# argmaxinc/DiffusionKit

Hardware: AMD Instinct MI355X
Metric: images/sec (whole node) FLUX.1-schnell 1024x1024 4-step (higher is better)
Workload: dtype bf16; 1 GPU; flux-schnell-1024: latent 128x128, 4 Euler steps, cfg_weight 0.0, text tokens 256, batch 1 image per GPU per step, + VAE decode to uint8; parallelism=dp1 (independent images, weight broadcast at load)

## Files before the change

### diffusionkit_amd/csrc/attention.hip

```cpp
#include "dk_kernels.h"

extern int g_dk_attn_mode;

static thread_local void* g_attn_ws = nullptr;
static thread_local size_t g_attn_ws_bytes = 0;
void dk_set_attention_workspace(void* ws, size_t bytes) { g_attn_ws = ws, g_attn_ws_bytes = ws ? bytes : 0; }
void* dk_get_attention_workspace() { return g_attn_ws; }
size_t dk_get_attention_workspace_bytes() { return g_attn_ws_bytes; }

int dk_launch_attention(const AttnParams& p_in, hipStream_t stream) {
  AttnParams p = p_in;
  if (p.bal_ws == nullptr) p.bal_ws = g_attn_ws;
  DK_REQUIRE(p.D == 128 || p.D == 64, "head_dim must be 64 or 128");
  DK_REQUIRE(p.S > 0 && p.B > 0 && p.H > 0, "empty attention");
  DK_REQUIRE(p.ld % 8 == 0 && p.ldo % 4 == 0, "row strides must keep 16-byte alignment");
  const long blocks5 = (long)p.B * p.H * ((p.S + 255) / 256);
  const bool long5 = p.D == 128 && (p.S >= 2048 || (p.S >= 1024 && blocks5 * 4 >= 3L * dk_device_cu_count()));
  int mode = p.bias != nullptr ? 4 : g_dk_attn_mode < 0 ? (long5 ? 10 : 4) : g_dk_attn_mode;
  if (mode == 10 && !dk_attention5_eligible(p)) mode = 9;
  dk_prof_begin(2, 4.0 * (double)p.B * p.H * (double)p.S * (double)p.S * p.D, stream);
  int rc = 0;
  switch (mode) {
    case 4: rc = dk_launch_attention2(p, 4, stream); break;
    case 9:
      rc = p.D == 128 ? dk_launch_attention4(p, stream) : dk_launch_attention2(p, 4, stream);
      break;
    case 10: rc = dk_launch_attention5(p, stream); break;
    default: DK_REQUIRE(false, "unknown attention variant (4: lean kernel, 9: phase-alternating kernel, 10: one-wave-per-SIMD kernel)");
  }
  dk_prof_end(stream);
  if (rc) return rc;
  DK_CHECK_HIP(hipGetLastError());
  if (p.O8 != nullptr && !((mode == 9 || mode == 10) && p.D == 128)) {
    Mx8Out o8{p.O8, p.O8_scales, p.o8_ld, p.o8_nblk, 0, p.B * p.S, 0, 0};
    return dk_launch_quantize_mx8(p.O, p.ldo, p.B * p.S, 0, p.B * p.S, p.H * p.D, o8, stream);
  }
  return 0;
}
```

### diffusionkit_amd/csrc/attention5.hip

```cpp
#include "dk_kernels.h"

typedef __attribute__((address_space(3))) char a5_lds_char;
typedef unsigned int u32x16 __attribute__((ext_vector_type(16)));
typedef unsigned int u32x8 __attribute__((ext_vector_type(8)));

#define A5_LDS_BYTES 131072

template <bool QFUSE>
__global__ __launch_bounds__(256, 1) void dk_attn5_fwd_kernel(AttnParams p) {
  constexpr int D = 128;
  extern __shared__ __attribute__((aligned(16))) char smem[];
  if ((unsigned)(size_t)(a5_lds_char*)smem != 0u) __builtin_trap();
  const int tid = threadIdx.x, lane = tid & 63;
  const int wave = __builtin_amdgcn_readfirstlane(tid >> 6);
  const int hi = lane >> 5, l31 = lane & 31;
  const int S = p.S;
  const int nq = (S + 255) / 256;
  auto xcd_contiguous = [](int bid, int nwg) {
    const int xcd = bid & 7, q = nwg >> 3, r = nwg & 7;
    return (xcd < r ? xcd * (q + 1) : r * (q + 1) + (xcd - r) * q) + (bid >> 3);
  };
  int t, part = 0, job = -1;
  if ((int)blockIdx.x < p.a5_whole) {
    t = xcd_contiguous(blockIdx.x, p.a5_whole);
  } else {
    job = xcd_contiguous(blockIdx.x - p.a5_whole, gridDim.x - p.a5_whole);
    t = p.a5_whole + job / p.a5_split;
    part = job % p.a5_split;
  }
  const unsigned row_bytes = (unsigned)p.ld * 2u;
  const int qblock = t % nq, head = (t / nq) % p.H, b = t / (nq * p.H);
  const int q0 = qblock * 256 + wave * 64;
  const int ng = S / 256, nparts = job < 0 ? 1 : p.a5_split;
  const int g_lo = (part * ng) / nparts, g_hi = ((part + 1) * ng) / nparts;
  const int tile0 = 4 * g_lo, nt = 4 * (g_hi - g_lo);

  const bf16_t* Qb = p.Q + (size_t)b * S * p.ld + head * D;
  const char* Kb = (const char*)(p.K + ((size_t)b * S + (size_t)tile0 * 64) * p.ld + head * D);
  const char* Vb = (const char*)(p.V + ((size_t)b * S + (size_t)tile0 * 64) * p.ld + head * D);

  u32x8 kaddr;
  const unsigned kr_base = (unsigned)(l31 * 256 + ((hi ^ (l31 & 15)) << 4));
#pragma unroll
  for (int kk = 0; kk < 8; ++kk) kaddr[kk] = kr_base ^ (unsigned)(kk << 5);
  const int x16 = (lane >> 4) & 1, p16 = lane & 15;
  u32x2 vaddr;
#pragma unroll
  for (int par = 0; par < 2; ++par) vaddr[par] = (unsigned)(65536 + x16 * 2048 + ((4 * (hi ^ x16) + (p16 >> 2)) ^ (2 * par + x16)) * 32 + (p16 & 3) * 8);
  u32x4 dk, dv;
#pragma unroll
  for (int i = 0; i < 4; ++i) {
    const int pi = 4 * wave + i;
    const int row = 4 * pi + (lane >> 4);
    dk[i] = (unsigned)row * row_bytes + (unsigned)(((lane & 15) ^ (row & 15)) << 4);
    const int dg = pi >> 1, hf = pi & 1;
    const int kl = (hf * 32 + (lane >> 1)) ^ (((dg & 1) << 2) | (dg & 3));
    dv[i] = (unsigned)kl * row_bytes + (unsigned)((2 * dg + (lane & 1)) << 4);
  }
  const u32x4 rK = {(unsigned)(size_t)Kb, (unsigned)((size_t)Kb >> 32) & 0xffffu, 0xffffffffu, 0x00020000u};
  const u32x4 rV = {(unsigned)(size_t)Vb, (unsigned)((size_t)Vb >> 32) & 0xffffu, 0xffffffffu, 0x00020000u};
  asm volatile(
#include "attention5_dma.inc"
      :
      : [tileb] "s"(64 * (int)row_bytes), [dbase] "s"(wave * 4096), "{v[248:251]}"(dk), "{v[252:255]}"(dv), "{s[40:43]}"(rK), "{s[44:47]}"(rV)
      : "s48", "s49", "s50", "s55", "m0", "scc", "memory");

  u32x16 qv[4];
#pragma unroll
  for (int qb = 0; qb < 2; ++qb) {
    bf16x8 qf[D / 16];
    const int qrow = min(q0 + qb * 32 + l31, S - 1);
    const bf16_t* qp = Qb + (size_t)qrow * p.ld + hi * 8;
#pragma unroll
    for (int kk = 0; kk < D / 16; ++kk) qf[kk] = *(const bf16x8*)(qp + kk * 16);
    if (QFUSE) {
      bf16x8 wv[D / 16];
      f32x4 t0[D / 16], t1[D / 16];
      if (p.qn_a != nullptr) {
        const bf16_t* w = (qrow < p.qn_split ? p.qn_a : p.qn_b) + hi * 8;
#pragma unroll
        for (int kk = 0; kk < D / 16; ++kk) wv[kk] = *(const bf16x8*)(w + kk * 16);
      }
      if (p.q_rope != nullptr) {
        const float* tab = p.q_rope + ((size_t)qrow * (D / 2) + hi * 4) * 2;
#pragma unroll
        for (int kk = 0; kk < D / 16; ++kk) t0[kk] = *(const f32x4*)(tab + kk * 16), t1[kk] = *(const f32x4*)(tab + kk * 16 + 4);
      }
      float v[D / 16][8];
#pragma unroll
      for (int kk = 0; kk < D / 16; ++kk)
#pragma unroll
        for (int e = 0; e < 8; ++e) v[kk][e] = (float)qf[kk][e];
      if (p.qn_a != nullptr) {
        float ss = 0.f;
#pragma unroll
        for (int kk = 0; kk < D / 16; ++kk)
#pragma unroll
          for (int e = 0; e < 8; ++e) ss += v[kk][e] * v[kk][e];
        ss += __shfl_xor(ss, 32, 64);
        const float r = rsqrtf(ss / (float)D + p.qn_eps);
#pragma unroll
        for (int kk = 0; kk < D / 16; ++kk)
#pragma unroll
          for (int e = 0; e < 8; ++e) v[kk][e] = round_bf16(v[kk][e] * r * (float)wv[kk][e]);
      }
      if (p.q_rope != nullptr) {
#pragma unroll
        for (int kk = 0; kk < D / 16; ++kk) {
          const float cs[8] = {t0[kk][0], t0[kk][1], t0[kk][2], t0[kk][3], t1[kk][0], t1[kk][1], t1[kk][2], t1[kk][3]};
#pragma unroll
          for (int i = 0; i < 4; ++i) {
            const float c = cs[2 * i], sn = cs[2 * i + 1], xe = v[kk][2 * i], xo = v[kk][2 * i + 1];
            v[kk][2 * i] = c * xe - sn * xo;
            v[kk][2 * i + 1] = sn * xe + c * xo;
          }
        }
      }
#pragma unroll
      for (int kk = 0; kk < D / 16; ++kk)
#pragma unroll
        for (int e = 0; e < 8; ++e) qf[kk][e] = (__bf16)v[kk][e];
    }
#pragma unroll
    for (int kk = 0; kk < D / 16; ++kk) {
      const u32x4 w4 = __builtin_bit_cast(u32x4, qf[kk]);
#pragma unroll
      for (int r = 0; r < 4; ++r) qv[(qb * 8 + kk) >> 2][((qb * 8 + kk) & 3) * 4 + r] = w4[r];
    }
  }

  const int scale_bits = __float_as_int(p.scale);

  f32x16 o[2][4];
  u32x2 lsum, mcv;
  asm volatile(
#include "attention5_asm.inc"
      : "={v[0:15]}"(o[0][0]), "={v[16:31]}"(o[0][1]), "={v[32:47]}"(o[0][2]), "={v[48:63]}"(o[0][3]), "={v[64:79]}"(o[1][0]), "={v[80:95]}"(o[1][1]),
        "={v[96:111]}"(o[1][2]), "={v[112:127]}"(o[1][3]), "={v[226:227]}"(lsum), "={v[224:225]}"(mcv), "+{v[128:143]}"(qv[0]), "+{v[144:159]}"(qv[1]), "+{v[160:175]}"(qv[2]),
        "+{v[176:191]}"(qv[3])
      : [koff] "s"(64 * (int)row_bytes), [voff] "s"(0), [tileb] "s"(64 * (int)row_bytes), [scale] "s"(scale_bits), [ntrip] "s"((nt - 8) / 4), [dbase] "s"(wave * 4096), "{v[238:245]}"(kaddr),
        "{v[246:247]}"(vaddr), "{v[248:251]}"(dk), "{v[252:255]}"(dv), "{s[40:43]}"(rK), "{s[44:47]}"(rV)
      :
#include "attention5_clobbers.inc"
  );

  int lane_t;
  asm volatile("v_mbcnt_lo_u32_b32 %0, -1, 0\n\tv_mbcnt_hi_u32_b32 %0, -1, %0" : "=v"(lane_t));
  {
    const int lane = lane_t, hi = lane >> 5, l31 = lane & 31;
#pragma unroll
  for (int qb = 0; qb < 2; ++qb) {
    const float l_run = __uint_as_float(lsum[qb]);
    const float inv = 1.0f / (l_run + __shfl_xor(l_run, 32, 64));
    const int q = q0 + qb * 32 + l31;
    if (p.O8 != nullptr) {
      const size_t orow = (size_t)b * S + min(q, S - 1);
#pragma unroll
      for (int dt = 0; dt < D / 32; ++dt) {
        float v[16], amax = 0.f;
#pragma unroll
        for (int e = 0; e < 16; ++e) {
          v[e] = round_bf16(o[qb][dt][e] * inv);
          amax = fmaxf(amax, fabsf(v[e]));
        }
        amax = fmaxf(amax, __shfl_xor(amax, 32, 64));
        const float ts = amax * (1.0f / 448.0f);
        unsigned e8 = (__float_as_uint(ts) + 0x7FFFFFu) >> 23;
        e8 = e8 < 1u ? 1u : (e8 > 254u ? 254u : e8);
        const float sc = __uint_as_float((254u - e8) << 23);
        if (q < S) {
          unsigned char* orow8 = p.O8 + orow * (size_t)p.o8_ld + head * D + dt * 32 + 4 * hi;
#pragma unroll
          for (int g4 = 0; g4 < 4; ++g4) {
            int w = 0;
            w = __builtin_amdgcn_cvt_pk_fp8_f32(v[4 * g4 + 0] * sc, v[4 * g4 + 1] * sc, w, false);
            w = __builtin_amdgcn_cvt_pk_fp8_f32(v[4 * g4 + 2] * sc, v[4 * g4 + 3] * sc, w, true);
            *(int*)(orow8 + 8 * g4) = w;
          }
          if (hi == 0) p.O8_scales[dk_mx_scale_index((unsigned)orow, (unsigned)(head * (D / 32) + dt), (unsigned)p.o8_nblk)] = (unsigned char)e8;
        }
      }
    }
  }
  if (p.O8 == nullptr) {
    a5_lds_char* const lds = (a5_lds_char*)0;
    const unsigned img = (unsigned)wave * 16384u;
#pragma unroll
    for (int qb = 0; qb < 2; ++qb) {
      const float l_run = __uint_as_float(lsum[qb]);
      const float inv = 1.0f / (l_run + __shfl_xor(l_run, 32, 64));
      const int r = qb * 32 + l31;
#pragma unroll
      for (int dt = 0; dt < D / 32; ++dt)
#pragma unroll
        for (int g4 = 0; g4 < 4; ++g4) {
          u32x2 w;
          w[0] = pack2bf(o[qb][dt][4 * g4 + 0] * inv, o[qb][dt][4 * g4 + 1] * inv);
          w[1] = pack2bf(o[qb][dt][4 * g4 + 2] * inv, o[qb][dt][4 * g4 + 3] * inv);
          *(__attribute__((address_space(3))) u32x2*)(lds + img + r * 256 + (((dt * 4 + g4) ^ (r & 15)) << 4) + hi * 8) = w;
        }
    }
    const int njobs = (int)gridDim.x - p.a5_whole;
    bf16_t* const ob = job < 0 ? p.O + ((size_t)b * S + q0) * p.ldo + head * D : (bf16_t*)p.a5_ws + ((size_t)job * 256 + wave * 64) * D;
    const size_t ldo = job < 0 ? (size_t)p.ldo : (size_t)D;
#pragma unroll
    for (int i = 0; i < 16; ++i) {
      const int r = 4 * i + (lane >> 4), pos = lane & 15;
      const u32x4 v = *(const __attribute__((address_space(3))) u32x4*)(lds + img + r * 256 + (pos << 4));
      if (q0 + r < S) *(u32x4*)(ob + (size_t)r * ldo + ((pos ^ (r & 15)) << 3)) = v;
    }
    if (job >= 0) {
      float* st = (float*)((char*)p.a5_ws + (size_t)njobs * 65536) + ((size_t)job * 256 + wave * 64) * 2;
#pragma unroll
      for (int qb = 0; qb < 2; ++qb) {
        const float l_run = __uint_as_float(lsum[qb]);
        const float l_row = l_run + __shfl_xor(l_run, 32, 64);
        if (hi == 0) *(f32x2*)(st + (qb * 32 + l31) * 2) = f32x2{__uint_as_float(mcv[qb]), l_row};
      }
    }
  }
  }
}

__global__ __launch_bounds__(256) void dk_attn5_merge_kernel(AttnParams p, int njobs) {
  constexpr int D = 128;
  const int blk = blockIdx.x >> 4, row = (blockIdx.x & 15) * 16 + (threadIdx.x >> 4), c8 = threadIdx.x & 15;
  const int nq = (p.S + 255) / 256;
  const int t = p.a5_whole + blk;
  const int qblock = t % nq, head = (t / nq) % p.H, b = t / (nq * p.H);
  const int q = qblock * 256 + row;
  const float* st = (const float*)((const char*)p.a5_ws + (size_t)njobs * 65536);
  float mc[4], l[4], mx = -3.0e38f;
  for (int i = 0; i < p.a5_split; ++i) {
    const f32x2 s2 = *(const f32x2*)(st + ((size_t)(blk * p.a5_split + i) * 256 + row) * 2);
    mc[i] = s2[0], l[i] = s2[1];
    mx = fmaxf(mx, mc[i]);
  }
  float acc[8] = {0.f, 0.f, 0.f, 0.f, 0.f, 0.f, 0.f, 0.f}, wsum = 0.f;
  for (int i = 0; i < p.a5_split; ++i) {
    const float w = l[i] * __builtin_amdgcn_exp2f(mc[i] - mx);
    const u32x4 v = *(const u32x4*)((const bf16_t*)p.a5_ws + ((size_t)(blk * p.a5_split + i) * 256 + row) * D + c8 * 8);
    wsum += w;
#pragma unroll
    for (int e = 0; e < 4; ++e) {
      float lo, hi2;
      unpack2bf(v[e], lo, hi2);
      acc[2 * e] += w * lo, acc[2 * e + 1] += w * hi2;
    }
  }
  const float inv = 1.0f / wsum;
  if (q < p.S) {
    u32x4 o;
#pragma unroll
    for (int e = 0; e < 4; ++e) o[e] = pack2bf(acc[2 * e] * inv, acc[2 * e + 1] * inv);
    *(u32x4*)(p.O + ((size_t)b * p.S + q) * p.ldo + head * D + c8 * 8) = o;
  }
}

int g_dk_attn5_split = -1;

bool dk_attention5_eligible(const AttnParams& p) {
  return p.D == 128 && p.bias == nullptr && p.S % 256 == 0 && p.S >= 12 * 64 && (size_t)p.S * p.ld * 2 < (1ull << 32);
}

int dk_launch_attention5(const AttnParams& p_in, hipStream_t stream) {
  DK_REQUIRE(dk_attention5_eligible(p_in), "attention5: head_dim 128, no score bias, S a multiple of 256 and >= 768");
  AttnParams p = p_in;
  const bool qfuse = p.qn_a != nullptr || p.q_rope != nullptr;
  if (qfuse) DK_REQUIRE(p.qn_a == nullptr || p.qn_b != nullptr, "qn_b missing (pass qn_a twice for one weight)");
  const int n_cu = dk_device_cu_count();
  const int nb = ((p.S + 255) / 256) * p.H * p.B;
  const int tail = nb % n_cu;
  int split = 1;
  if (tail > 0 && p.O8 == nullptr && g_dk_attn5_split != 0) {
    for (int s = 2; s <= 4 && split == 1; ++s) {
      if ((p.S / 256) / s < 3) break;
      if (g_dk_attn5_split > 0 ? s == g_dk_attn5_split : (tail * s <= n_cu && tail * s * 10 >= n_cu * 6)) split = s;
    }
    void* ws = dk_get_attention_workspace();
    if (split > 1 && (ws == nullptr || dk_get_attention_workspace_bytes() < (size_t)tail * split * (65536 + 2048))) split = 1;
    p.a5_ws = ws;
  }
  p.a5_split = split;
  p.a5_whole = split > 1 ? nb - tail : nb;
  const int njobs = split > 1 ? tail * split : 0;
  static DkDeviceOnce attr_once;
  if (attr_once.first()) {
    DK_CHECK_HIP(hipFuncSetAttribute((const void*)dk_attn5_fwd_kernel<true>, hipFuncAttributeMaxDynamicSharedMemorySize, A5_LDS_BYTES));
    DK_CHECK_HIP(hipFuncSetAttribute((const void*)dk_attn5_fwd_kernel<false>, hipFuncAttributeMaxDynamicSharedMemorySize, A5_LDS_BYTES));
    attr_once.mark();
  }
  if (qfuse)
    hipLaunchKernelGGL((dk_attn5_fwd_kernel<true>), dim3((unsigned)(p.a5_whole + njobs)), dim3(256), A5_LDS_BYTES, stream, p);
  else
    hipLaunchKernelGGL((dk_attn5_fwd_kernel<false>), dim3((unsigned)(p.a5_whole + njobs)), dim3(256), A5_LDS_BYTES, stream, p);
  if (njobs > 0) hipLaunchKernelGGL(dk_attn5_merge_kernel, dim3((unsigned)(tail * 16)), dim3(256), 0, stream, p, njobs);
  return 0;
}
```

### diffusionkit_amd/csrc/dk_kernels.h

```cpp
#pragma once
#include "../../include/dk_hip.h"
#include "dk_common.h"
#include "dk_ksplit.h"


struct GemmParams {
  const bf16_t* A;
  const bf16_t* W;
  bf16_t* C;
  const bf16_t* bias;
  const bf16_t* gate;
  const bf16_t* res;
  int M, N, K;
  int lda, ldc, ldr;
  int ldw;
  int a_seg_len, a_seg_stride;
  int c_seg_len, c_seg_stride;
  int r_seg_len, r_seg_stride;
  int gate_seg_len, gate_stride;
  float alpha;
  int epi;
  int conv;
  int cB, cH, cW, cC, ups;
  const bf16_t* zeros;
// ... 58 lines not shown
}

struct GemmF8Params {
  const unsigned char* A;
  const unsigned char* SA;
  const unsigned char* W;
  const float* wscale;
  void* C;
  const bf16_t* bias;
  const bf16_t* gate;
  const bf16_t* res;
  int M, N, K;
  int lda, ldw, ldc, ldr;
  int a_seg_len, a_seg_stride, a_row0;
  int sa_nblk;
  int c_seg_len, c_seg_stride;
  int r_seg_len, r_seg_stride;
  int gate_seg_len, gate_stride;
  int epi;
  int c_mx8;
  int n_split;
  void* C2;
  int ldc2, epi2, c2_mx8;
  unsigned char* SC;
  int sc_nblk, c_row0, sc_kb0;
  const bf16_t* kn_w;
  const float* kn_rope;
  int kn_col0, kn_col1, kn_D, kn_pos_off, kn_seg_len;
  float kn_eps;
  const bf16_t* qn_w;
  int qn_col0, qn_col1;
  void* workspace;
  size_t workspace_bytes;
};
bool dk_gemm256f8_eligible(const GemmF8Params& p);
int dk_launch_gemm256f8(const GemmF8Params& p, const GemmF8Params* p2, hipStream_t stream);
struct Mx8Out {
  unsigned char* out;
  unsigned char* scales;
  int ldo, n_blk128, row0, seg_len, seg_stride, col0;
};
int dk_launch_quantize_mx8(const bf16_t* x, int ldx, int x_seg_len, int x_seg_stride, int M, int h, const Mx8Out& o, hipStream_t stream);
int dk_launch_ln_modulate_mx8(const bf16_t* x, int ldx, int M, int h, const bf16_t* shift, const bf16_t* scale, int mod_stride, int seg_len,
                              int x_seg_len, int x_seg_stride, float eps, const Mx8Out& o, hipStream_t stream);
int dk_launch_ln_modulate2_mx8(const bf16_t* x0, int M0, const bf16_t* shift0, const bf16_t* scale0, int seg0, const Mx8Out& o0,
                               const bf16_t* x1, int M1, const bf16_t* shift1, const bf16_t* scale1, int seg1, const Mx8Out& o1, int ldx, int h,
                               int mod_stride, int x_seg_stride, float eps, hipStream_t stream);

void dk_prof_begin(int cls, double work, hipStream_t st);
void dk_prof_end(hipStream_t st);

struct AttnParams {
  const bf16_t* Q;
  const bf16_t* K;
  const bf16_t* V;
  bf16_t* O;
  int B, H, S, D;
  int ld, ldo;
  float scale;
  const bf16_t* bias = nullptr;
  long bias_head_stride = 0;
  int ldb = 0;
  const bf16_t* qn_a = nullptr;
  const bf16_t* qn_b = nullptr;
  int qn_split = 0;
  float qn_eps = 1e-6f;
  const float* q_rope = nullptr;
  void* bal_ws = nullptr;
  unsigned char* O8 = nullptr;
  unsigned char* O8_scales = nullptr;
  int o8_ld = 0, o8_nblk = 0;
  int a5_whole = 0, a5_split = 1;
  void* a5_ws = nullptr;
};
void dk_set_attention_workspace(void* ws, size_t bytes = 0);
void* dk_get_attention_workspace();
size_t dk_get_attention_workspace_bytes();
extern int g_dk_attn_mode;
int dk_launch_attention(const AttnParams& p, hipStream_t stream);
int dk_launch_attention2(const AttnParams& p, int waves, hipStream_t stream);
int dk_launch_attention4(const AttnParams& p, hipStream_t stream);
bool dk_attention5_eligible(const AttnParams& p);
int dk_launch_attention5(const AttnParams& p, hipStream_t stream);
extern int g_dk_attn5_split;

struct Attn512Params {
  const bf16_t* Q;
  const bf16_t* K;
  const bf16_t* Vt;
  bf16_t* O;
  int T, Tp, B, ld, ldo;
  float scale;
};
int dk_launch_attention512(const Attn512Params& p, hipStream_t stream);

int dk_launch_embedding(const bf16_t* table, const int* ids, const bf16_t* pos, int pos_rows, bf16_t* out, float* out_f32, int n, int dim,
                        int vocab, hipStream_t stream);
int dk_launch_layernorm(const bf16_t* x, bf16_t* out, int M, int h, const bf16_t* w, const bf16_t* b, float eps, hipStream_t stream);
int dk_launch_t5_rmsnorm(const float* x, bf16_t* out, int M, int h, const bf16_t* w, float eps, hipStream_t stream);
int dk_launch_text_elementwise(const bf16_t* a, const bf16_t* b, bf16_t* y, float* r, long n, int op, hipStream_t stream);
int dk_launch_t5_bias(const bf16_t* emb, const int* rel_bucket, int H, int S, int ld, bf16_t* out, hipStream_t stream);

int dk_launch_ln_modulate(const bf16_t* x, int ldx, bf16_t* out, int ldo, int M, int h,
                          const bf16_t* shift, const bf16_t* scale, int mod_stride, int seg_len,
                          int x_seg_len, int x_seg_stride, float eps, hipStream_t stream);
int dk_launch_qk_norm_rope(bf16_t* qkv, int ld, int q_off, int k_off, int rows, int H, int D,
                           const bf16_t* qw, const bf16_t* kw, float eps, const float* rope,
                           int row_seg_len, int row_seg_stride, int pos_off, int S_pos,
                           hipStream_t stream, int k_only = 0);
int dk_launch_ln_modulate2(const bf16_t* x0, bf16_t* out0, int M0, const bf16_t* shift0, const bf16_t* scale0, int seg0, const bf16_t* x1,
                           bf16_t* out1, int M1, const bf16_t* shift1, const bf16_t* scale1, int seg1, int ldx, int ldo, int h,
                           int mod_stride, int x_seg_stride, float eps, hipStream_t stream);
int dk_launch_qk_norm_rope2(bf16_t* qkv0, int rows0, const bf16_t* qw0, const bf16_t* kw0, int seg0, int pos0, bf16_t* qkv1, int rows1,
                            const bf16_t* qw1, const bf16_t* kw1, int seg1, int pos1, int ld, int q_off, int k_off, int H, int D,
                            float eps, const float* rope, int row_seg_stride, hipStream_t stream, int k_only = 0);
int dk_launch_silu(const bf16_t* x, bf16_t* y, long n, hipStream_t stream);
int dk_launch_add(const bf16_t* a, const bf16_t* b, int b_rows, bf16_t* y, int rows, int cols, hipStream_t stream);
int dk_launch_timestep_embedding(const float* t, int n, int rep, int dim, float max_period, int embed_dtype,
                                 bf16_t* out, hipStream_t stream);
int dk_launch_rope_table(float* table, int S_txt, int gh, int gw, const int* axes, int n_axes, float theta,
                         hipStream_t stream);
int dk_launch_f32_to_bf16(const float* x, bf16_t* y, long n, hipStream_t stream);
int dk_launch_affine_f32(const float* x, float* y, long n, float a, float b, hipStream_t stream);
int dk_launch_latent_to_tokens(const float* x, bf16_t* tok, int n_img, int dup, int Hl, int Wl, int C, int p,
                               int reshape_order, hipStream_t stream);
int dk_launch_euler_step(float* x, const bf16_t* model_out, int ld_out, bf16_t* tok, int n_img, int cfg_on,
                         int Hl, int Wl, int C, int p, int reshape_order, float sigma, float sigma_next,
                         float cfg_weight, hipStream_t stream);

struct ConvHaloParams {
  const bf16_t* x;
  const bf16_t* w;
  const bf16_t* bias;
  const bf16_t* bias2;
  const bf16_t* res;
  bf16_t* y;
  const float* gn_ss;
  int gn_silu;
  const bf16_t* x2;
  int C2;
  float* stats_out;
  int G_out;
  float* img;
  unsigned char* u8;
  bf16_t* raw;
  int out_channels;
  int B, H, W, C, O, ups, ldw, ldy, ldr;
};
bool dk_conv_halo_eligible(const ConvHaloParams& p, bool img);
int dk_launch_conv_halo(const ConvHaloParams& p, hipStream_t stream);
extern int g_dk_conv_v4;
bool dk_conv256v4_eligible(const ConvHaloParams& p);
bool dk_conv256v4_wanted(const ConvHaloParams& p);
int dk_launch_conv256v4(const ConvHaloParams& p, hipStream_t stream);

int dk_launch_groupnorm_finalize(const float* partial, int nchunk, int B, int G, double count, float eps, float* mean_rstd,
                                 const bf16_t* gamma, const bf16_t* beta, int C, float* scale_shift, hipStream_t stream);
int dk_launch_groupnorm_partials(const bf16_t* x, int B, long HW, int C, int G, float* partial, int nchunk, hipStream_t stream);
int dk_launch_groupnorm_stats(const bf16_t* x, int B, long HW, int C, int G, float* partial, int nchunk,
                              float* mean_rstd, float eps, hipStream_t stream);
int dk_launch_groupnorm_apply(const bf16_t* x, bf16_t* y, int B, long HW, int C, int G, const float* mean_rstd,
                              const bf16_t* gamma, const bf16_t* beta, int do_silu, hipStream_t stream);
int dk_launch_softmax_rows(bf16_t* x, int rows, int cols, int ld, hipStream_t stream);
int dk_launch_transpose(const bf16_t* x, bf16_t* y, int R, int Cc, hipStream_t stream, int ldy = 0);
int dk_launch_pad_channels(const float* x, bf16_t* y, long npix, int C, int Cpad, hipStream_t stream);
int dk_launch_image_post(const bf16_t* x, int ldx, float* img, unsigned char* u8, long npix, hipStream_t stream);
int dk_launch_latent_sample(const bf16_t* mom, int ldm, const float* noise, float* out, long npix, int L, hipStream_t stream);
// ... 2 lines not shown
```

### diffusionkit_amd/csrc/engine.hip

```cpp
#include <hip/hip_runtime.h>

#include <cmath>
#include <cstdio>
#include <cstring>
#include <type_traits>
#include <string>
#include <unordered_map>
#include <vector>

#include "../../include/dk_hip.h"
#include "dk_kernels.h"

static thread_local std::string g_last_error;
void dk_set_error(const std::string& msg) { g_last_error = msg; }

extern "C" int dk_abi_version(void) { return DK_ABI_VERSION; }
extern "C" const char* dk_last_error(void) { return g_last_error.c_str(); }

int g_dk_attn_mode = -1;
int g_dk_fuse_k = 1;
int g_dk_fuse_qg = -1;
int g_dk_fuse_q = 1;
int g_dk_pitch_min_k = 8192;
int g_dk_conv_halo = -1;
extern "C" int32_t dk_weight_pitch(int32_t k) { return k >= g_dk_pitch_min_k ? k + 64 : k; }
extern "C" int dk_tune_set(const char* key, int32_t value) {
  DK_REQUIRE(key != nullptr, "null key");
  if (strcmp(key, "gemm") == 0) { g_dk_gemm_mode = value; return 0; }
  if (strcmp(key, "gemm_v4") == 0) { g_dk_v4_auto = value; return 0; }
  if (strcmp(key, "gemm_skew") == 0) { g_dk_v4_skew = value; return 0; }
  if (strcmp(key, "attn") == 0) { g_dk_attn_mode = value; return 0; }
  if (strcmp(key, "attn_fuse_q") == 0) { g_dk_fuse_q = value; return 0; }
  if (strcmp(key, "attn_split") == 0) { g_dk_attn5_split = value; return 0; }
  if (strcmp(key, "gemm_fuse_k") == 0) { g_dk_fuse_k = value; return 0; }
  if (strcmp(key, "gemm_fuse_q") == 0) { g_dk_fuse_qg = value; return 0; }
  if (strcmp(key, "gemm_split") == 0) { g_dk_v3_split = value; return 0; }
  if (strcmp(key, "gemm_split_min") == 0) { g_dk_v3_split_min = value; return 0; }
  if (strcmp(key, "gemm_pair_nk") == 0) { g_dk_pair_split_nk = value; return 0; }
  if (strcmp(key, "gemm_mf") == 0) { g_dk_v3_mf = value; return 0; }
  if (strcmp(key, "pitch_min_k") == 0) { g_dk_pitch_min_k = value; return 0; }
  if (strcmp(key, "conv_halo") == 0) { g_dk_conv_halo = value; return 0; }
  if (strcmp(key, "conv_v4") == 0) { g_dk_conv_v4 = value; return 0; }
  dk_set_error(std::string("unknown tuning key: ") + key);
  return -1;
}

static inline hipStream_t S_(void* s) { return (hipStream_t)s; }
static inline size_t align_up(size_t v, size_t a) { return (v + a - 1) / a * a; }

static GemmParams gemm_params_from_desc(const dk_gemm_desc* d) {
  GemmParams p;
  memset(&p, 0, sizeof(p));
  p.A = (const bf16_t*)d->A; p.W = (const bf16_t*)d->W; p.C = (bf16_t*)d->C;
  p.bias = (const bf16_t*)d->bias; p.gate = (const bf16_t*)d->gate; p.res = (const bf16_t*)d->res;
  p.M = d->M; p.N = d->N; p.K = d->K;
  p.lda = d->lda; p.ldc = d->ldc; p.ldr = d->ldr;
  p.a_seg_len = d->a_seg_len > 0 ? d->a_seg_len : d->M; p.a_seg_stride = d->a_seg_stride;
  p.c_seg_len = d->c_seg_len > 0 ? d->c_seg_len : d->M; p.c_seg_stride = d->c_seg_stride;
  p.r_seg_len = d->r_seg_len > 0 ? d->r_seg_len : d->M; p.r_seg_stride = d->r_seg_stride;
  p.gate_seg_len = d->gate_seg_len > 0 ? d->gate_seg_len : d->M; p.gate_stride = d->gate_stride;
  p.alpha = d->alpha; p.epi = d->epilogue; p.ldw = d->ldw;
  p.workspace = d->workspace; p.workspace_bytes = d->workspace_bytes;
  return p;
}

extern "C" size_t dk_gemm_workspace_bytes(void) { return dk_gemm_split_workspace_bytes(); }

extern "C" int dk_gemm_bf16(const dk_gemm_desc* d, void* stream) {
  DK_REQUIRE(d != nullptr, "null descriptor");
  return dk_launch_gemm(gemm_params_from_desc(d), S_(stream));
}

extern "C" int dk_gemm_plan(const dk_gemm_desc* d, const dk_gemm_desc* d2, dk_gemm_plan_t* plan) {
  DK_REQUIRE(d != nullptr && plan != nullptr, "null descriptor / plan");
  const GemmParams p2 = d2 != nullptr ? gemm_params_from_desc(d2) : GemmParams{};
  return dk_gemm_plan_call(gemm_params_from_desc(d), d2 != nullptr ? &p2 : nullptr, *plan);
}

template <class P, class F>
static void set_fused(P& p, const F* f) {
  if (f == nullptr) return;
  p.n_split = f->n_split; p.C2 = (decltype(p.C2))f->C2; p.ldc2 = f->ldc2; p.epi2 = f->epi2;
  p.kn_w = (const bf16_t*)f->kn_w; p.kn_rope = f->kn_rope;
  p.kn_col0 = f->kn_col0; p.kn_col1 = f->kn_col1; p.kn_D = f->kn_D; p.kn_pos_off = f->kn_pos_off; p.kn_seg_len = f->kn_seg_len; p.kn_eps = f->kn_eps;
  p.qn_w = (const bf16_t*)f->qn_w; p.qn_col0 = f->qn_col0; p.qn_col1 = f->qn_col1;
}

extern "C" int dk_gemm_fused_bf16(const dk_gemm_desc* d, const dk_gemm_side* f, const dk_gemm_desc* d2, const dk_gemm_side* f2, void* stream) {
  DK_REQUIRE(d != nullptr && (d2 != nullptr || f2 == nullptr), "null descriptor");
  GemmParams p = gemm_params_from_desc(d);
  set_fused(p, f);
  if (d2 == nullptr) return dk_launch_gemm(p, S_(stream));
  GemmParams p2 = gemm_params_from_desc(d2);
  set_fused(p2, f2);
  return dk_launch_gemm_pair(p, p2, S_(stream));
}

extern "C" int dk_gemm_fused_plan(const dk_gemm_desc* d, const dk_gemm_side* f, const dk_gemm_desc* d2, const dk_gemm_side* f2,
                                  dk_gemm_plan_t* plan) {
  DK_REQUIRE(d != nullptr && plan != nullptr && (d2 != nullptr || f2 == nullptr), "null descriptor / plan");
  GemmParams p = gemm_params_from_desc(d), p2 = d2 != nullptr ? gemm_params_from_desc(d2) : GemmParams{};
  set_fused(p, f);
  if (d2 != nullptr) set_fused(p2, f2);
  return dk_gemm_plan_call(p, d2 != nullptr ? &p2 : nullptr, *plan);
}

static int conv3x3_launch(const dk_conv_desc* d, void* workspace, hipStream_t stream) {
  DK_REQUIRE(d != nullptr, "null descriptor");
  GemmParams p;
  memset(&p, 0, sizeof(p));
  p.A = (const bf16_t*)d->x; p.W = (const bf16_t*)d->w; p.C = (bf16_t*)d->y;
  p.bias = (const bf16_t*)d->bias; p.res = (const bf16_t*)d->res;
  p.M = d->B * d->H * d->W; p.N = d->O; p.K = 9 * d->C;
  p.lda = d->C; p.ldc = d->ldy; p.ldr = d->ldr;
  p.a_seg_len = p.c_seg_len = p.r_seg_len = p.gate_seg_len = p.M;
  p.alpha = 1.0f; p.epi = d->epilogue;
// ... 1368 lines not shown
```

Before: 4.109 images/s.

## Make attention5 kernel persistent, overlapping next tile's K/Q loads with output store

```diff
diff --git a/diffusionkit_amd/csrc/attention.hip b/diffusionkit_amd/csrc/attention.hip
--- a/diffusionkit_amd/csrc/attention.hip
+++ b/diffusionkit_amd/csrc/attention.hip
@@ -15,7 +15,7 @@
   DK_REQUIRE(p.S > 0 && p.B > 0 && p.H > 0, "empty attention");
   DK_REQUIRE(p.ld % 8 == 0 && p.ldo % 4 == 0, "row strides must keep 16-byte alignment");
   const long blocks5 = (long)p.B * p.H * ((p.S + 255) / 256);
-  const bool long5 = p.D == 128 && (p.S >= 2048 || (p.S >= 1024 && blocks5 * 4 >= 3L * dk_device_cu_count()));
+  const bool long5 = p.D == 128 && (p.S >= 2048 || (p.S >= 1024 && dk_attention5_eligible(p) && blocks5 * 4 >= 3L * dk_device_cu_count()));
   int mode = p.bias != nullptr ? 4 : g_dk_attn_mode < 0 ? (long5 ? 10 : 4) : g_dk_attn_mode;
   if (mode == 10 && !dk_attention5_eligible(p)) mode = 9;
   dk_prof_begin(2, 4.0 * (double)p.B * p.H * (double)p.S * (double)p.S * p.D, stream);
diff --git a/diffusionkit_amd/csrc/attention5.hip b/diffusionkit_amd/csrc/attention5.hip
--- a/diffusionkit_amd/csrc/attention5.hip
+++ b/diffusionkit_amd/csrc/attention5.hip
@@ -11,214 +11,292 @@
   constexpr int D = 128;
   extern __shared__ __attribute__((aligned(16))) char smem[];
   if ((unsigned)(size_t)(a5_lds_char*)smem != 0u) __builtin_trap();
-  const int tid = threadIdx.x, lane = tid & 63;
-  const int wave = __builtin_amdgcn_readfirstlane(tid >> 6);
-  const int hi = lane >> 5, l31 = lane & 31;
-  const int S = p.S;
+  const int wave = __builtin_amdgcn_readfirstlane(threadIdx.x >> 6);
+  typedef const __attribute__((address_space(4))) AttnParams* a5_params_ptr;
+  auto params = []() {
+    a5_params_ptr q = (a5_params_ptr)__builtin_amdgcn_kernarg_segment_ptr();
+    asm volatile("" : "+s"(q));
+    return q;
+  };
+  a5_params_ptr P = params();
+  const int S = P->S;
   const int nq = (S + 255) / 256;
-  auto xcd_contiguous = [](int bid, int nwg) {
-    const int xcd = bid & 7, q = nwg >> 3, r = nwg & 7;
-    return (xcd < r ? xcd * (q + 1) : r * (q + 1) + (xcd - r) * q) + (bid >> 3);
-  };
-  int t, part = 0, job = -1;
-  if ((int)blockIdx.x < p.a5_whole) {
-    t = xcd_contiguous(blockIdx.x, p.a5_whole);
+  const int njobs = (nq * P->H * P->B - P->a5_whole) * P->a5_split;
+  const int nwg = (int)gridDim.x - njobs;
+  auto xcd_first = [](int xcd, int n) {
+    const int q = n >> 3, r = n & 7;
+    return xcd < r ? xcd * (q + 1) : r * (q + 1) + (xcd - r) * q;
+  };
+  int t, t_end, t_step, part = 0, job = -1;
+  if ((int)blockIdx.x < nwg) {
+    const int xcd = blockIdx.x & 7;
+    t = xcd_first(xcd, P->a5_whole) + (blockIdx.x >> 3);
+    t_end = xcd_first(xcd + 1, P->a5_whole);
+    t_step = (nwg - xcd + 7) >> 3;
   } else {
-    job = xcd_contiguous(blockIdx.x - p.a5_whole, gridDim.x - p.a5_whole);
-    t = p.a5_whole + job / p.a5_split;
-    part = job % p.a5_split;
-  }
-  const unsigned row_bytes = (unsigned)p.ld * 2u;
-  const int qblock = t % nq, head = (t / nq) % p.H, b = t / (nq * p.H);
-  const int q0 = qblock * 256 + wave * 64;
-  const int ng = S / 256, nparts = job < 0 ? 1 : p.a5_split;
+    job = xcd_first((blockIdx.x - nwg) & 7, njobs) + ((blockIdx.x - nwg) >> 3);
+    t = P->a5_whole + job / P->a5_split;
+    part = job % P->a5_split;
+    t_end = t + 1, t_step = 1;
+  }
+  const unsigned row_bytes = (unsigned)P->ld * 2u;
+  const int ng = S / 256, nparts = job < 0 ? 1 : P->a5_split;
   const int g_lo = (part * ng) / nparts, g_hi = ((part + 1) * ng) / nparts;
   const int tile0 = 4 * g_lo, nt = 4 * (g_hi - g_lo);
 
-  const bf16_t* Qb = p.Q + (size_t)b * S * p.ld + head * D;
-  const char* Kb = (const char*)(p.K + ((size_t)b * S + (size_t)tile0 * 64) * p.ld + head * D);
-  const char* Vb = (const char*)(p.V + ((size_t)b * S + (size_t)tile0 * 64) * p.ld + head * D);
-
-  u32x8 kaddr;
-  const unsigned kr_base = (unsigned)(l31 * 256 + ((hi ^ (l31 & 15)) << 4));
-#pragma unroll
-  for (int kk = 0; kk < 8; ++kk) kaddr[kk] = kr_base ^ (unsigned)(kk << 5);
-  const int x16 = (lane >> 4) & 1, p16 = lane & 15;
-  u32x2 vaddr;
-#pragma unroll
-  for (int par = 0; par < 2; ++par) vaddr[par] = (unsigned)(65536 + x16 * 2048 + ((4 * (hi ^ x16) + (p16 >> 2)) ^ (2 * par + x16)) * 32 + (p16 & 3) * 8);
-  u32x4 dk, dv;
-#pragma unroll
-  for (int i = 0; i < 4; ++i) {
-    const int pi = 4 * wave + i;
-    const int row = 4 * pi + (lane >> 4);
-    dk[i] = (unsigned)row * row_bytes + (unsigned)(((lane & 15) ^ (row & 15)) << 4);
-    const int dg = pi >> 1, hf = pi & 1;
-    const int kl = (hf * 32 + (lane >> 1)) ^ (((dg & 1) << 2) | (dg & 3));
-    dv[i] = (unsigned)kl * row_bytes + (unsigned)((2 * dg + (lane & 1)) << 4);
-  }
-  const u32x4 rK = {(unsigned)(size_t)Kb, (unsigned)((size_t)Kb >> 32) & 0xffffu, 0xffffffffu, 0x00020000u};
-  const u32x4 rV = {(unsigned)(size_t)Vb, (unsigned)((size_t)Vb >> 32) & 0xffffu, 0xffffffffu, 0x00020000u};
-  asm volatile(
+  auto sgpr = [](int v) { return __builtin_amdgcn_readfirstlane(v); };
+  auto other_half = [](float v, int lane) { return __int_as_float(__builtin_amdgcn_ds_bpermute((lane ^ 32) << 2, __float_as_int(v))); };
+  auto fresh_lane = []() {
+    int l;
+    asm volatile("v_mbcnt_lo_u32_b32 %0, -1, 0\n\tv_mbcnt_hi_u32_b32 %0, -1, %0" : "=v"(l));
+    return l;
+  };
+  auto piece_offsets = [&](int lane, u32x4& dk, u32x4& dv) {
+#pragma unroll
+    for (int i = 0; i < 4; ++i) {
+      const int pi = 4 * wave + i;
+      const int row = 4 * pi + (lane >> 4);
+      dk[i] = (unsigned)row * row_bytes + (unsigned)(((lane & 15) ^ (row & 15)) << 4);
+      const int dg = pi >> 1, hf = pi & 1;
+      const int kl = (hf * 32 + (lane >> 1)) ^ (((dg & 1) << 2) | (dg & 3));
+      dv[i] = (unsigned)kl * row_bytes + (unsigned)((2 * dg + (lane & 1)) << 4);
+    }
+  };
+  auto kv_resource = [&](const bf16_t* base, int tb) {
+    const int head = sgpr((tb / nq) % P->H), b = sgpr(tb / (nq * P->H));
+    const char* a = (const char*)(base + ((size_t)b * S + (size_t)tile0 * 64) * P->ld + head * D);
+    return u32x4{(unsigned)sgpr((int)(size_t)a), (unsigned)sgpr((int)((size_t)a >> 32)) & 0xffffu, 0xffffffffu, 0x00020000u};
+  };
+  auto issue_k0 = [&](int tb, int lane) {
+    u32x4 dk, dv;
+    piece_offsets(lane, dk, dv);
+    const u32x4 rK = kv_resource(P->K, tb), rV = kv_resource(P->V, tb);
+    asm volatile(
 #include "attention5_dma.inc"
-      :
-      : [tileb] "s"(64 * (int)row_bytes), [dbase] "s"(wave * 4096), "{v[248:251]}"(dk), "{v[252:255]}"(dv), "{s[40:43]}"(rK), "{s[44:47]}"(rV)
-      : "s48", "s49", "s50", "s55", "m0", "scc", "memory");
-
-  u32x16 qv[4];
-#pragma unroll
-  for (int qb = 0; qb < 2; ++qb) {
-    bf16x8 qf[D / 16];
-    const int qrow = min(q0 + qb * 32 + l31, S - 1);
-    const bf16_t* qp = Qb + (size_t)qrow * p.ld + hi * 8;
-#pragma unroll
-    for (int kk = 0; kk < D / 16; ++kk) qf[kk] = *(const bf16x8*)(qp + kk * 16);
-    if (QFUSE) {
-      bf16x8 wv[D / 16];
-      f32x4 t0[D / 16], t1[D / 16];
-      if (p.qn_a != nullptr) {
-        const bf16_t* w = (qrow < p.qn_split ? p.qn_a : p.qn_b) + hi * 8;
-#pragma unroll
-        for (int kk = 0; kk < D / 16; ++kk) wv[kk] = *(const bf16x8*)(w + kk * 16);
-      }
-      if (p.q_rope != nullptr) {
-        const float* tab = p.q_rope + ((size_t)qrow * (D / 2) + hi * 4) * 2;
-#pragma unroll
-        for (int kk = 0; kk < D / 16; ++kk) t0[kk] = *(const f32x4*)(tab + kk * 16), t1[kk] = *(const f32x4*)(tab + kk * 16 + 4);
-      }
-      float v[D / 16][8];
-#pragma unroll
-      for (int kk = 0; kk < D / 16; ++kk)
-#pragma unroll
-        for (int e = 0; e < 8; ++e) v[kk][e] = (float)qf[kk][e];
-      if (p.qn_a != nullptr) {
-        float ss = 0.f;
+        :
+        : [tileb] "s"(64 * (int)row_bytes), [dbase] "s"(wave * 4096), "{v[248:251]}"(dk), "{v[252:255]}"(dv), "{s[40:43]}"(rK), "{s[44:47]}"(rV)
+        : "s48", "s49", "s50", "s55", "m0", "scc", "memory");
+  };
+  auto q_row = [&](int tb, int qb, int lane) { return min(sgpr(tb % nq) * 256 + wave * 64 + qb * 32 + (lane & 31), S - 1); };
+  auto load_q = [&](int tb, int lane, bf16x8 (&qf)[2][D / 16]) {
+    const int head = sgpr((tb / nq) % P->H), b = sgpr(tb / (nq * P->H));
+#pragma unroll
+    for (int qb = 0; qb < 2; ++qb) {
+      const bf16_t* qp = P->Q + (size_t)b * S * P->ld + head * D + (size_t)q_row(tb, qb, lane) * P->ld + (lane >> 5) * 8;
+#pragma unroll
+      for (int kk = 0; kk < D / 16; ++kk) qf[qb][kk] = *(const bf16x8*)(qp + kk * 16);
+    }
+  };
+  auto make_qv = [&](int tb, int lane, bf16x8 (&qf)[2][D / 16], unsigned (&qw)[64]) {
+    const int hi = lane >> 5;
+#pragma unroll
+    for (int qb = 0; qb < 2; ++qb) {
+      if (QFUSE) {
+        bf16x8 wv[D / 16];
+        f32x4 t0[D / 16], t1[D / 16];
+        const int qrow = q_row(tb, qb, lane);
+        if (P->qn_a != nullptr) {
+          const bf16_t* w = (qrow < P->qn_split ? P->qn_a : P->qn_b) + hi * 8;
+#pragma unroll
+          for (int kk = 0; kk < D / 16; ++kk) wv[kk] = *(const bf16x8*)(w + kk * 16);
+        }
+        if (P->q_rope != nullptr) {
+          const float* tab = P->q_rope + ((size_t)qrow * (D / 2) + hi * 4) * 2;
+#pragma unroll
+          for (int kk = 0; kk < D / 16; ++kk) t0[kk] = *(const f32x4*)(tab + kk * 16), t1[kk] = *(const f32x4*)(tab + kk * 16 + 4);
+        }
+        float v[D / 16][8];
 #pragma unroll
         for (int kk = 0; kk < D / 16; ++kk)
 #pragma unroll
-          for (int e = 0; e < 8; ++e) ss += v[kk][e] * v[kk][e];
-        ss += __shfl_xor(ss, 32, 64);
-        const float r = rsqrtf(ss / (float)D + p.qn_eps);
+          for (int e = 0; e < 8; ++e) v[kk][e] = (float)qf[qb][kk][e];
+        if (P->qn_a != nullptr) {
+          float ss = 0.f;
+#pragma unroll
+          for (int kk = 0; kk < D / 16; ++kk)
+#pragma unroll
+            for (int e = 0; e < 8; ++e) ss += v[kk][e] * v[kk][e];
+          ss += other_half(ss, lane);
+          const float r = rsqrtf(ss / (float)D + P->qn_eps);
+#pragma unroll
+          for (int kk = 0; kk < D / 16; ++kk)
+#pragma unroll
+            for (int e = 0; e < 8; ++e) v[kk][e] = round_bf16(v[kk][e] * r * (float)wv[kk][e]);
+        }
+        if (P->q_rope != nullptr) {
+#pragma unroll
+          for (int kk = 0; kk < D / 16; ++kk) {
+            const float cs[8] = {t0[kk][0], t0[kk][1], t0[kk][2], t0[kk][3], t1[kk][0], t1[kk][1], t1[kk][2], t1[kk][3]};
+#pragma unroll
+            for (int i = 0; i < 4; ++i) {
+              const float c = cs[2 * i], sn = cs[2 * i + 1], xe = v[kk][2 * i], xo = v[kk][2 * i + 1];
+              v[kk][2 * i] = c * xe - sn * xo;
+              v[kk][2 * i + 1] = sn * xe + c * xo;
+            }
+          }
+        }
 #pragma unroll
         for (int kk = 0; kk < D / 16; ++kk)
 #pragma unroll
-          for (int e = 0; e < 8; ++e) v[kk][e] = round_bf16(v[kk][e] * r * (float)wv[kk][e]);
-      }
-      if (p.q_rope != nullptr) {
-#pragma unroll
-        for (int kk = 0; kk < D / 16; ++kk) {
-          const float cs[8] = {t0[kk][0], t0[kk][1], t0[kk][2], t0[kk][3], t1[kk][0], t1[kk][1], t1[kk][2], t1[kk][3]};
-#pragma unroll
-          for (int i = 0; i < 4; ++i) {
-            const float c = cs[2 * i], sn = cs[2 * i + 1], xe = v[kk][2 * i], xo = v[kk][2 * i + 1];
-            v[kk][2 * i] = c * xe - sn * xo;
-            v[kk][2 * i + 1] = sn * xe + c * xo;
+          for (int e = 0; e < 8; ++e) qf[qb][kk][e] = (__bf16)v[kk][e];
+      }
+#pragma unroll
+      for (int kk = 0; kk < D / 16; ++kk) {
+        const u32x4 w4 = __builtin_bit_cast(u32x4, qf[qb][kk]);
+#pragma unroll
+        for (int r = 0; r < 4; ++r) qw[(qb * 8 + kk) * 4 + r] = w4[r];
+      }
+    }
+  };
+  auto lds_addresses = [&](int lane, unsigned (&ad)[18]) {
+    const int hi = lane >> 5, l31 = lane & 31;
+    const unsigned kr_base = (unsigned)(l31 * 256 + ((hi ^ (l31 & 15)) << 4));
+#pragma unroll
+    for (int kk = 0; kk < 8; ++kk) ad[kk] = kr_base ^ (unsigned)(kk << 5);
+    const int x16 = (lane >> 4) & 1, p16 = lane & 15;
+#pragma unroll
+    for (int par = 0; par < 2; ++par) ad[8 + par] = (unsigned)(65536 + x16 * 2048 + ((4 * (hi ^ x16) + (p16 >> 2)) ^ (2 * par + x16)) * 32 + (p16 & 3) * 8);
+    u32x4 dk, dv;
+    piece_offsets(lane, dk, dv);
+#pragma unroll
+    for (int i = 0; i < 4; ++i) ad[10 + i] = dk[i], ad[14 + i] = dv[i];
+  };
+
+  auto tile_loop = [&](int tb, int lane, bf16x8 (&qf)[2][D / 16], f32x16 (&o)[2][4], u32x2& lsum, u32x2& mcv) {
+    unsigned qw[64], ad[18];
+    make_qv(tb, lane, qf, qw);
+    lds_addresses(lane, ad);
+    u32x16 qv[4];
+    u32x8 kaddr;
+    u32x2 vaddr;
+    u32x4 dk, dv;
+#pragma unroll
+    for (int i = 0; i < 64; ++i) qv[i >> 4][i & 15] = qw[i];
+#pragma unroll
+    for (int i = 0; i < 8; ++i) kaddr[i] = ad[i];
+#pragma unroll
+    for (int i = 0; i < 4; ++i) dk[i] = ad[10 + i], dv[i] = ad[14 + i];
+    vaddr[0] = ad[8], vaddr[1] = ad[9];
+    const u32x4 rK = kv_resource(P->K, t), rV = kv_resource(P->V, t);
+    const int scale_bits = __float_as_int(P->scale);
+    asm volatile(
+#include "attention5_asm.inc"
+        : "={v[0:15]}"(o[0][0]), "={v[16:31]}"(o[0][1]), "={v[32:47]}"(o[0][2]), "={v[48:63]}"(o[0][3]), "={v[64:79]}"(o[1][0]), "={v[80:95]}"(o[1][1]),
+          "={v[96:111]}"(o[1][2]), "={v[112:127]}"(o[1][3]), "={v[226:227]}"(lsum), "={v[224:225]}"(mcv), "+{v[128:143]}"(qv[0]), "+{v[144:159]}"(qv[1]), "+{v[160:175]}"(qv[2]),
+          "+{v[176:191]}"(qv[3])
+        : [koff] "s"(64 * (int)row_bytes), [voff] "s"(0), [tileb] "s"(64 * (int)row_bytes), [scale] "s"(scale_bits), [ntrip] "s"((nt - 8) / 4), [dbase] "s"(wave * 4096), "{v[238:245]}"(kaddr),
+          "{v[246:247]}"(vaddr), "{v[248:251]}"(dk), "{v[252:255]}"(dv), "{s[40:43]}"(rK), "{s[44:47]}"(rV)
+        :
+#include "attention5_clobbers.inc"
+    );
+  };
+  auto store_block = [&](int tb, int lane, f32x16 (&o)[2][4], u32x2& lsum, u32x2& mcv) {
+    const int qblock = sgpr(tb % nq), head = sgpr((tb / nq) % P->H), b = sgpr(tb / (nq * P->H));
+    const int q0 = qblock * 256 + wave * 64;
+  {
+    const int hi = lane >> 5, l31 = lane & 31;
+    if (P->O8 != nullptr) {
+#pragma unroll
+      for (int qb = 0; qb < 2; ++qb) {
+        const float l_run = __uint_as_float(lsum[qb]);
+        const float inv = 1.0f / (l_run + other_half(l_run, lane));
+        const int q = q0 + qb * 32 + l31;
+        const size_t orow = (size_t)b * S + min(q, S - 1);
+#pragma unroll
+        for (int dt = 0; dt < D / 32; ++dt) {
+          float v[16], amax = 0.f;
+#pragma unroll
+          for (int e = 0; e < 16; ++e) {
+            v[e] = round_bf16(o[qb][dt][e] * inv);
+            amax = fmaxf(amax, fabsf(v[e]));
           }
-        }
-      }
-#pragma unroll
-      for (int kk = 0; kk < D / 16; ++kk)
-#pragma unroll
-        for (int e = 0; e < 8; ++e) qf[kk][e] = (__bf16)v[kk][e];
-    }
-#pragma unroll
-    for (int kk = 0; kk < D / 16; ++kk) {
-      const u32x4 w4 = __builtin_bit_cast(u32x4, qf[kk]);
-#pragma unroll
-      for (int r = 0; r < 4; ++r) qv[(qb * 8 + kk) >> 2][((qb * 8 + kk) & 3) * 4 + r] = w4[r];
-    }
-  }
-
-  const int scale_bits = __float_as_int(p.scale);
+          amax = fmaxf(amax, other_half(amax, lane));
+          const float ts = amax * (1.0f / 448.0f);
+          unsigned e8 = (__float_as_uint(ts) + 0x7FFFFFu) >> 23;
+          e8 = e8 < 1u ? 1u : (e8 > 254u ? 254u : e8);
+          const float sc = __uint_as_float((254u - e8) << 23);
+          if (q < S) {
+            unsigned char* orow8 = P->O8 + orow * (size_t)P->o8_ld + head * D + dt * 32 + 4 * hi;
+#pragma unroll
+            for (int g4 = 0; g4 < 4; ++g4) {
+              int w = 0;
+              w = __builtin_amdgcn_cvt_pk_fp8_f32(v[4 * g4 + 0] * sc, v[4 * g4 + 1] * sc, w, false);
+              w = __builtin_amdgcn_cvt_pk_fp8_f32(v[4 * g4 + 2] * sc, v[4 * g4 + 3] * sc, w, true);
+              *(int*)(orow8 + 8 * g4) = w;
+            }
+            if (hi == 0) {
+              const unsigned kb = (unsigned)(head * (D / 32) + dt), r = (unsigned)orow;
+              unsigned char* const sc_base = P->O8_scales + (((size_t)(kb >> 2) * (unsigned)P->o8_nblk * 64) << 3);
+              sc_base[((((r >> 7) * 64 + (kb & 3) * 16 + (r & 15)) << 3) + ((r >> 4) & 7))] = (unsigned char)e8;
+            }
+          }
+        }
+      }
+    } else {
+      a5_lds_char* const lds = (a5_lds_char*)0;
+      const unsigned img = 65536u + (unsigned)wave * 16384u;
+#pragma unroll
+      for (int qb = 0; qb < 2; ++qb) {
+        const float l_run = __uint_as_float(lsum[qb]);
+        const float inv = 1.0f / (l_run + other_half(l_run, lane));
+        const int r = qb * 32 + l31;
+#pragma unroll
+        for (int dt = 0; dt < D / 32; ++dt)
+#pragma unroll
+          for (int g4 = 0; g4 < 4; ++g4) {
+            u32x2 w;
+            w[0] = pack2bf(o[qb][dt][4 * g4 + 0] * inv, o[qb][dt][4 * g4 + 1] * inv);
+            w[1] = pack2bf(o[qb][dt][4 * g4 + 2] * inv, o[qb][dt][4 * g4 + 3] * inv);
+            *(__attribute__((address_space(3))) u32x2*)(lds + img + r * 256 + (((dt * 4 + g4) ^ (r & 15)) << 4) + hi * 8) = w;
+          }
+      }
+      bf16_t* const ob = job < 0 ? P->O + ((size_t)b * S + q0) * P->ldo + head * D : (bf16_t*)P->a5_ws + ((size_t)job * 256 + wave * 64) * D;
+      const size_t ldo = job < 0 ? (size_t)P->ldo : (size_t)D;
+#pragma unroll
+      for (int i = 0; i < 16; ++i) {
+        const int r = 4 * i + (lane >> 4), pos = lane & 15;
+        const u32x4 v = *(const __attribute__((address_space(3))) u32x4*)(lds + img + r * 256 + (pos << 4));
+        if (q0 + r < S) *(u32x4*)(ob + (size_t)r * ldo + ((pos ^ (r & 15)) << 3)) = v;
+      }
+      if (job >= 0) {
+        float* st = (float*)((char*)P->a5_ws + (size_t)njobs * 65536) + ((size_t)job * 256 + wave * 64) * 2;
+#pragma unroll
+        for (int qb = 0; qb < 2; ++qb) {
+          const float l_run = __uint_as_float(lsum[qb]);
+          const float l_row = l_run + other_half(l_run, lane);
+          if (hi == 0) *(f32x2*)(st + (qb * 32 + l31) * 2) = f32x2{__uint_as_float(mcv[qb]), l_row};
+        }
+      }
+    }
+  }
+  };
 
   f32x16 o[2][4];
   u32x2 lsum, mcv;
-  asm volatile(
-#include "attention5_asm.inc"
-      : "={v[0:15]}"(o[0][0]), "={v[16:31]}"(o[0][1]), "={v[32:47]}"(o[0][2]), "={v[48:63]}"(o[0][3]), "={v[64:79]}"(o[1][0]), "={v[80:95]}"(o[1][1]),
-        "={v[96:111]}"(o[1][2]), "={v[112:127]}"(o[1][3]), "={v[226:227]}"(lsum), "={v[224:225]}"(mcv), "+{v[128:143]}"(qv[0]), "+{v[144:159]}"(qv[1]), "+{v[160:175]}"(qv[2]),
-        "+{v[176:191]}"(qv[3])
-      : [koff] "s"(64 * (int)row_bytes), [voff] "s"(0), [tileb] "s"(64 * (int)row_bytes), [scale] "s"(scale_bits), [ntrip] "s"((nt - 8) / 4), [dbase] "s"(wave * 4096), "{v[238:245]}"(kaddr),
-        "{v[246:247]}"(vaddr), "{v[248:251]}"(dk), "{v[252:255]}"(dv), "{s[40:43]}"(rK), "{s[44:47]}"(rV)
-      :
-#include "attention5_clobbers.inc"
-  );
-
-  int lane_t;
-  asm volatile("v_mbcnt_lo_u32_b32 %0, -1, 0\n\tv_mbcnt_hi_u32_b32 %0, -1, %0" : "=v"(lane_t));
   {
-    const int lane = lane_t, hi = lane >> 5, l31 = lane & 31;
-#pragma unroll
-  for (int qb = 0; qb < 2; ++qb) {
-    const float l_run = __uint_as_float(lsum[qb]);
-    const float inv = 1.0f / (l_run + __shfl_xor(l_run, 32, 64));
-    const int q = q0 + qb * 32 + l31;
-    if (p.O8 != nullptr) {
-      const size_t orow = (size_t)b * S + min(q, S - 1);
-#pragma unroll
-      for (int dt = 0; dt < D / 32; ++dt) {
-        float v[16], amax = 0.f;
-#pragma unroll
-        for (int e = 0; e < 16; ++e) {
-          v[e] = round_bf16(o[qb][dt][e] * inv);
-          amax = fmaxf(amax, fabsf(v[e]));
-        }
-        amax = fmaxf(amax, __shfl_xor(amax, 32, 64));
-        const float ts = amax * (1.0f / 448.0f);
-        unsigned e8 = (__float_as_uint(ts) + 0x7FFFFFu) >> 23;
-        e8 = e8 < 1u ? 1u : (e8 > 254u ? 254u : e8);
-        const float sc = __uint_as_float((254u - e8) << 23);
-        if (q < S) {
-          unsigned char* orow8 = p.O8 + orow * (size_t)p.o8_ld + head * D + dt * 32 + 4 * hi;
-#pragma unroll
-          for (int g4 = 0; g4 < 4; ++g4) {
-            int w = 0;
-            w = __builtin_amdgcn_cvt_pk_fp8_f32(v[4 * g4 + 0] * sc, v[4 * g4 + 1] * sc, w, false);
-            w = __builtin_amdgcn_cvt_pk_fp8_f32(v[4 * g4 + 2] * sc, v[4 * g4 + 3] * sc, w, true);
-            *(int*)(orow8 + 8 * g4) = w;
-          }
-          if (hi == 0) p.O8_scales[dk_mx_scale_index((unsigned)orow, (unsigned)(head * (D / 32) + dt), (unsigned)p.o8_nblk)] = (unsigned char)e8;
-        }
-      }
-    }
-  }
-  if (p.O8 == nullptr) {
-    a5_lds_char* const lds = (a5_lds_char*)0;
-    const unsigned img = (unsigned)wave * 16384u;
-#pragma unroll
-    for (int qb = 0; qb < 2; ++qb) {
-      const float l_run = __uint_as_float(lsum[qb]);
-      const float inv = 1.0f / (l_run + __shfl_xor(l_run, 32, 64));
-      const int r = qb * 32 + l31;
-#pragma unroll
-      for (int dt = 0; dt < D / 32; ++dt)
-#pragma unroll
-        for (int g4 = 0; g4 < 4; ++g4) {
-          u32x2 w;
-          w[0] = pack2bf(o[qb][dt][4 * g4 + 0] * inv, o[qb][dt][4 * g4 + 1] * inv);
-          w[1] = pack2bf(o[qb][dt][4 * g4 + 2] * inv, o[qb][dt][4 * g4 + 3] * inv);
-          *(__attribute__((address_space(3))) u32x2*)(lds + img + r * 256 + (((dt * 4 + g4) ^ (r & 15)) << 4) + hi * 8) = w;
-        }
-    }
-    const int njobs = (int)gridDim.x - p.a5_whole;
-    bf16_t* const ob = job < 0 ? p.O + ((size_t)b * S + q0) * p.ldo + head * D : (bf16_t*)p.a5_ws + ((size_t)job * 256 + wave * 64) * D;
-    const size_t ldo = job < 0 ? (size_t)p.ldo : (size_t)D;
-#pragma unroll
-    for (int i = 0; i < 16; ++i) {
-      const int r = 4 * i + (lane >> 4), pos = lane & 15;
-      const u32x4 v = *(const __attribute__((address_space(3))) u32x4*)(lds + img + r * 256 + (pos << 4));
-      if (q0 + r < S) *(u32x4*)(ob + (size_t)r * ldo + ((pos ^ (r & 15)) << 3)) = v;
-    }
-    if (job >= 0) {
-      float* st = (float*)((char*)p.a5_ws + (size_t)njobs * 65536) + ((size_t)job * 256 + wave * 64) * 2;
-#pragma unroll
-      for (int qb = 0; qb < 2; ++qb) {
-        const float l_run = __uint_as_float(lsum[qb]);
-        const float l_row = l_run + __shfl_xor(l_run, 32, 64);
-        if (hi == 0) *(f32x2*)(st + (qb * 32 + l31) * 2) = f32x2{__uint_as_float(mcv[qb]), l_row};
-      }
-    }
-  }
+    bf16x8 qf[2][D / 16];
+    const int lane = fresh_lane();
+    issue_k0(t, lane);
+    load_q(t, lane, qf);
+    tile_loop(t, lane, qf, o, lsum, mcv);
+  }
+  for (;;) {
+    const int lane = fresh_lane();
+    P = params();
+    const int t_next = t + t_step;
+    if (t_next >= t_end) break;
+    bf16x8 qf[2][D / 16];
+    issue_k0(t_next, lane);
+    load_q(t_next, lane, qf);
+    store_block(t, lane, o, lsum, mcv);
+    asm volatile("s_waitcnt lgkmcnt(0)\n\ts_barrier" ::: "memory");
+    t = t_next;
+    tile_loop(t, lane, qf, o, lsum, mcv);
+  }
+  {
+    const int lane = fresh_lane();
+    P = params();
+    store_block(t, lane, o, lsum, mcv);
   }
 }
 
@@ -258,6 +336,7 @@
 }
 
 int g_dk_attn5_split = -1;
+int g_dk_attn5_persist = -1;
 
 bool dk_attention5_eligible(const AttnParams& p) {
   return p.D == 128 && p.bias == nullptr && p.S % 256 == 0 && p.S >= 12 * 64 && (size_t)p.S * p.ld * 2 < (1ull << 32);
@@ -284,6 +363,8 @@
   p.a5_split = split;
   p.a5_whole = split > 1 ? nb - tail : nb;
   const int njobs = split > 1 ? tail * split : 0;
+  const bool persist = g_dk_attn5_persist != 0;
+  const int nwg = persist && p.a5_whole > n_cu ? n_cu : p.a5_whole;
   static DkDeviceOnce attr_once;
   if (attr_once.first()) {
     DK_CHECK_HIP(hipFuncSetAttribute((const void*)dk_attn5_fwd_kernel<true>, hipFuncAttributeMaxDynamicSharedMemorySize, A5_LDS_BYTES));
@@ -291,9 +372,9 @@
     attr_once.mark();
   }
   if (qfuse)
-    hipLaunchKernelGGL((dk_attn5_fwd_kernel<true>), dim3((unsigned)(p.a5_whole + njobs)), dim3(256), A5_LDS_BYTES, stream, p);
+    hipLaunchKernelGGL((dk_attn5_fwd_kernel<true>), dim3((unsigned)(nwg + njobs)), dim3(256), A5_LDS_BYTES, stream, p);
   else
-    hipLaunchKernelGGL((dk_attn5_fwd_kernel<false>), dim3((unsigned)(p.a5_whole + njobs)), dim3(256), A5_LDS_BYTES, stream, p);
+    hipLaunchKernelGGL((dk_attn5_fwd_kernel<false>), dim3((unsigned)(nwg + njobs)), dim3(256), A5_LDS_BYTES, stream, p);
   if (njobs > 0) hipLaunchKernelGGL(dk_attn5_merge_kernel, dim3((unsigned)(tail * 16)), dim3(256), 0, stream, p, njobs);
   return 0;
 }
diff --git a/diffusionkit_amd/csrc/dk_kernels.h b/diffusionkit_amd/csrc/dk_kernels.h
--- a/diffusionkit_amd/csrc/dk_kernels.h
+++ b/diffusionkit_amd/csrc/dk_kernels.h
@@ -164,7 +164,7 @@
 int dk_launch_attention4(const AttnParams& p, hipStream_t stream);
 bool dk_attention5_eligible(const AttnParams& p);
 int dk_launch_attention5(const AttnParams& p, hipStream_t stream);
-extern int g_dk_attn5_split;
+extern int g_dk_attn5_split, g_dk_attn5_persist;
 
 struct Attn512Params {
   const bf16_t* Q;
diff --git a/diffusionkit_amd/csrc/engine.hip b/diffusionkit_amd/csrc/engine.hip
--- a/diffusionkit_amd/csrc/engine.hip
+++ b/diffusionkit_amd/csrc/engine.hip
@@ -32,6 +32,7 @@
   if (strcmp(key, "attn") == 0) { g_dk_attn_mode = value; return 0; }
   if (strcmp(key, "attn_fuse_q") == 0) { g_dk_fuse_q = value; return 0; }
   if (strcmp(key, "attn_split") == 0) { g_dk_attn5_split = value; return 0; }
+  if (strcmp(key, "attn_persist") == 0) { g_dk_attn5_persist = value; return 0; }
   if (strcmp(key, "gemm_fuse_k") == 0) { g_dk_fuse_k = value; return 0; }
   if (strcmp(key, "gemm_fuse_q") == 0) { g_dk_fuse_qg = value; return 0; }
   if (strcmp(key, "gemm_split") == 0) { g_dk_v3_split = value; return 0; }
```

Result: no change. 4.108 images/s (-0.0%).
